# rasd3/TODA

Measured on AMD Instinct MI355X. Metric: LiDAR training samples/sec, higher is better.
Workload: dtype f32

## Files before the change

toda_amd/csrc/spconv.hip:

```cpp
#include <stdlib.h>

#include <type_traits>

#include <hip/hip_ext.h>

#include <mutex>
#include <vector>

#include "bn_fold.cuh"
#include "common.h"


namespace toda {

typedef float f32x4 __attribute__((ext_vector_type(4)));

constexpr int SC_BLOCK = 256;

static int tiles_pow2(int channels) {
    int t = (channels + 15) / 16, p = 1;
    while (p < t) p <<= 1;
    return p;
}

__global__ void __launch_bounds__(SC_BLOCK)
pack_weight_kernel(const float* __restrict__ w, int cout, int K, int cin, int transpose, int flip_k, int Q, int NT,
                   float* __restrict__ wp) {
    const long long e = (long long)blockIdx.x * SC_BLOCK + threadIdx.x;
    const long long total = (long long)K * Q * NT * 256;
    if (e >= total) return;
    const int j = (int)(e & 3);
    const int lane = (int)((e >> 2) & 63);
    long long t = e >> 8;
    const int n = (int)(t % NT);
    t /= NT;
    const int q = (int)(t % Q);
    const int k = (int)(t / Q);
    const int c = lane & 15, g = lane >> 4;
    const int gch = 16 * q + 4 * g + j;
    const int pch = NT * c + n;
    const int kk = flip_k ? K - 1 - k : k;
    float v = 0.0f;
    if (!transpose) {
        if (gch < cin && pch < cout) v = w[((size_t)pch * K + kk) * cin + gch];
    } else {
        if (gch < cout && pch < cin) v = w[((size_t)gch * K + kk) * cin + pch];
    }
    wp[e] = v;
}

constexpr int PACK_MAX_SEG = 48;
struct PackBatch {
    const float* w[PACK_MAX_SEG];
    float* wp[PACK_MAX_SEG];
    int cout[PACK_MAX_SEG], K[PACK_MAX_SEG], cin[PACK_MAX_SEG];
    unsigned char transpose[PACK_MAX_SEG], flip[PACK_MAX_SEG], Q[PACK_MAX_SEG], NT[PACK_MAX_SEG];
};

__global__ void __launch_bounds__(SC_BLOCK)
pack_weight_batch_kernel(const PackBatch b) {
    const int sg = blockIdx.y;
    const int K = b.K[sg], Q = b.Q[sg], NT = b.NT[sg], cin = b.cin[sg], cout = b.cout[sg];
    const long long e = (long long)blockIdx.x * SC_BLOCK + threadIdx.x;
// ... 951 lines not shown
    PackBatch b = {};
    toda::SplitPackBatch sb = {};
    int m = 0, sm = 0;
    long long most = 0, smost = 0;
    auto flush = [&]() -> int {
        if (m > 0) {
            hipLaunchKernelGGL(pack_weight_batch_kernel, dim3(cdiv(most, SC_BLOCK), m), dim3(SC_BLOCK), 0, (hipStream_t)stream, b);
            TODA_LAUNCH_CHECK();
        }
        m = 0, most = 0;
        return TODA_OK;
    };
    auto sflush = [&]() -> int {
        if (sm > 0) {
            hipLaunchKernelGGL(split_pack_batch_kernel, dim3(cdiv(smost, SC_BLOCK), sm), dim3(SC_BLOCK), 0, (hipStream_t)stream, sb);
            TODA_LAUNCH_CHECK();
        }
        sm = 0, smost = 0;
        return TODA_OK;
    };
    for (int s = 0; s < n; ++s) {
        TODA_CHECK_ARG(w[s] && wp[s] && cout[s] >= 1 && cin[s] >= 1 && k_vol[s] >= 1, "pack_weights: bad segment %d", s);
        const int cgather = transpose[s] ? cout[s] : cin[s], cprod = transpose[s] ? cin[s] : cout[s];
        TODA_CHECK_ARG(cgather <= 128 && cprod <= 128, "pack_weights: channels > 128 unsupported (segment %d)", s);
        if (use_split(cgather, cprod)) {
            split_pack_fill(sb, sm, w[s], cout[s], k_vol[s], cin[s], transpose[s], flip_k[s], wp[s]);
            const long long total = (long long)k_vol[s] * sb.KC[sm] * sb.NT[sm] * 192;
            if (total > smost) smost = total;
            if (++sm == toda::SPLIT_PACK_MAX_SEG) {
                const int rc = sflush();
                if (rc != TODA_OK) return rc;
            }
            continue;
        }
        const int i = m;
        b.w[i] = w[s], b.wp[i] = wp[s], b.cout[i] = cout[s], b.K[i] = k_vol[s], b.cin[i] = cin[s];
        b.transpose[i] = transpose[s] != 0, b.flip[i] = flip_k[s] != 0;
        b.Q[i] = (unsigned char)tiles_pow2(cgather), b.NT[i] = (unsigned char)tiles_pow2(cprod);
        const long long total = (long long)k_vol[s] * b.Q[i] * b.NT[i] * 256;
        if (total > most) most = total;
        if (++m == PACK_MAX_SEG) {
            const int rc = flush();
            if (rc != TODA_OK) return rc;
        }
    }
    {
        const int rc = flush();
        if (rc != TODA_OK) return rc;
    }
    return sflush();
}

namespace toda {
constexpr int CLS_ROWS = 8192, CLS_PER = CLS_ROWS / 256;
struct ClassGeom {
    int stride[3], pad[3];
};
__global__ void __launch_bounds__(256)
class_order_kernel(const int4* __restrict__ coords, int n, const ClassGeom gm, int32_t* __restrict__ order, unsigned char* __restrict__ cls_sorted) {
    __shared__ int cnt[8][256 + 1];
    const int base = blockIdx.x * CLS_ROWS, t = threadIdx.x;
    unsigned char c[CLS_PER];
    int mine[8] = {0, 0, 0, 0, 0, 0, 0, 0};
#pragma unroll
    for (int i = 0; i < CLS_PER; ++i) {
        const int r = base + t * CLS_PER + i;
        int cl = 0;
        if (r < n) {
            const int4 v = coords[r];
            cl = (((v.y + gm.pad[0]) % gm.stride[0]) * gm.stride[1] + (v.z + gm.pad[1]) % gm.stride[1]) * gm.stride[2] + (v.w + gm.pad[2]) % gm.stride[2];
            ++mine[cl & 7];
        }
        c[i] = (unsigned char)cl;
    }
#pragma unroll
    for (int k = 0; k < 8; ++k) cnt[k][t] = mine[k];
    __syncthreads();
    if (t < 8) {
        int run = 0;
        for (int j = 0; j < 256; ++j) {
            const int v = cnt[t][j];
            cnt[t][j] = run;
            run += v;
        }
        cnt[t][256] = run;
    }
    __syncthreads();
    int cls_base[8], run = 0;
#pragma unroll
    for (int k = 0; k < 8; ++k) {
        cls_base[k] = run + cnt[k][t];
        run += cnt[k][256];
    }
#pragma unroll
    for (int i = 0; i < CLS_PER; ++i) {
        const int r = base + t * CLS_PER + i;
        if (r >= n) break;
        const int k = c[i] & 7;
        int pos = 0;
#pragma unroll
        for (int q = 0; q < 8; ++q)
            if (q == k) pos = cls_base[q]++;
        order[base + pos] = r;
        cls_sorted[base + pos] = c[i];
    }
}

static int class_table(const int32_t* ksize, const int32_t* stride, const int32_t* pad, GatherClasses* out) {
    const int n_class = stride[0] * stride[1] * stride[2];
    if (n_class < 1 || n_class > 8 || ksize[0] * ksize[1] * ksize[2] > 27) return -1;
    *out = GatherClasses{};
    for (int rz = 0; rz < stride[0]; ++rz)
        for (int ry = 0; ry < stride[1]; ++ry)
            for (int rx = 0; rx < stride[2]; ++rx) {
                const int c = (rz * stride[1] + ry) * stride[2] + rx;
                int m = 0;
                for (int kz = 0; kz < ksize[0]; ++kz)
                    for (int ky = 0; ky < ksize[1]; ++ky)
                        for (int kx = 0; kx < ksize[2]; ++kx)
                            if (kz % stride[0] == rz && ky % stride[1] == ry && kx % stride[2] == rx)
                                out->k[c][m++] = (unsigned char)((kz * ksize[1] + ky) * ksize[2] + kx);
                out->count[c] = (unsigned char)m;
            }
    return 0;
}
}

extern "C" int toda_rulebook_class_order(const int32_t* in_coords, int n_in, const int32_t* stride, const int32_t* padding, int32_t* order,
                                         unsigned char* cls_sorted, void* stream) {
    TODA_CHECK_ARG(in_coords && stride && padding && order && cls_sorted && n_in >= 0, "rulebook_class_order: null argument");
    ClassGeom gm;
    for (int a = 0; a < 3; ++a) {
        TODA_CHECK_ARG(stride[a] >= 1 && stride[a] <= 2 && padding[a] >= 0, "rulebook_class_order: stride 1 or 2 per axis (got %d)", stride[a]);
        gm.stride[a] = stride[a], gm.pad[a] = padding[a];
    }
    if (n_in == 0) return TODA_OK;
    hipLaunchKernelGGL(class_order_kernel, dim3(cdiv(n_in, CLS_ROWS)), dim3(256), 0, (hipStream_t)stream, (const int4*)in_coords, n_in, gm, order,
                       cls_sorted);
    TODA_LAUNCH_CHECK();
    return TODA_OK;
}

namespace toda {
struct LaunchTimer {
    std::vector<hipEvent_t> ev;
    int used = 0;
    bool on = false;
};
static LaunchTimer g_timer;
static std::mutex g_timer_mu;
static inline void timer_next(hipEvent_t* start, hipEvent_t* stop) {
    *start = *stop = nullptr;
    if (!g_timer.on) return;
    std::lock_guard<std::mutex> lock(g_timer_mu);
    if (!g_timer.on || 2 * (g_timer.used + 1) > (int)g_timer.ev.size()) return;
    *start = g_timer.ev[2 * g_timer.used];
    *stop = g_timer.ev[2 * g_timer.used + 1];
    g_timer.used++;
}
}

#define GG_LAUNCH(kernel, grid, block, shmem, stream, ...)                                              \
    do {                                                                                               \
        hipEvent_t t0_, t1_;                                                                           \
        toda::timer_next(&t0_, &t1_);                                                                  \
        hipExtLaunchKernelGGL(kernel, grid, block, shmem, stream, t0_, t1_, 0, __VA_ARGS__);           \
    } while (0)

extern "C" int toda_timing_begin(int capacity) {
    TODA_CHECK_ARG(capacity > 0 && capacity <= (1 << 20), "timing_begin: capacity in (0, 2^20]");
    std::lock_guard<std::mutex> lock(toda::g_timer_mu);
    for (hipEvent_t e : g_timer.ev) (void)hipEventDestroy(e);
    g_timer.ev.assign((size_t)2 * capacity, nullptr);
    for (auto& e : g_timer.ev) TODA_HIP(hipEventCreate(&e));
    g_timer.used = 0;
    g_timer.on = true;
    return TODA_OK;
}

extern "C" int toda_timing_end(float* ms_out, int cap, int* n_out) {
    std::lock_guard<std::mutex> lock(toda::g_timer_mu);
    g_timer.on = false;
    const int n = g_timer.used < cap ? g_timer.used : cap;
    for (int i = 0; i < n; ++i) {
        TODA_HIP(hipEventSynchronize(g_timer.ev[2 * i + 1]));
        TODA_HIP(hipEventElapsedTime(&ms_out[i], g_timer.ev[2 * i], g_timer.ev[2 * i + 1]));
    }
    if (n_out) *n_out = g_timer.used;
    for (hipEvent_t e : g_timer.ev) (void)hipEventDestroy(e);
    g_timer.ev.clear();
// ... 28 lines not shown
    int rt, block, grid;
    bool vec;
};
}

static int gather_route(int c_gather, int c_produce, int n_out, bool stats, bool cls_sorted, GatherRoute* r) {
    const int Q = tiles_pow2(c_gather), NT = tiles_pow2(c_produce);
    const bool vec_ok = (c_gather & 3) == 0;
    const bool lds_faster = Q >= 2 && NT >= Q;
    r->rt = 2, r->block = SC_BLOCK, r->vec = vec_ok;
    if (use_split(c_gather, c_produce)) {
        TODA_CHECK_ARG(!(cls_sorted && stats), "gather_gemm (split path): no statistics on a class-sorted launch");
        r->family = GatherRoute::SPLIT;
    } else if (vec_ok && Q == 8 && NT == 8 && !cls_sorted) {
        r->family = GatherRoute::LDS_128, r->rt = 1, r->block = 512;
    } else if ((lds_faster || stats) && !cls_sorted && vec_ok && Q * NT <= 32) {
        r->family = GatherRoute::LDS, r->rt = NT < 8 ? 2 : 1;
    } else {
        TODA_CHECK_ARG(!stats, "gather_gemm: statistics requested on a launch shape without the fused epilogue");
        TODA_CHECK_ARG(vec_ok || Q == 1, "gather_gemm: gathered channel counts above 16 must be multiples of 4 (got %d)", c_gather);
        r->family = GatherRoute::REG;
        r->rt = NT < 8 ? 2 : (Q < 8 ? 1 : 2);
    }
    r->grid = cdiv(cdiv(n_out, 16 * r->rt), r->block / 64);
    return TODA_OK;
}

static int gather_gemm_impl(const float* in, int n_in, int c_gather, const float* wp, const int32_t* nbr, int n_out, int k_vol,
                            int c_produce, const float* bias, float* out, const int32_t* order, double* stats, int* blocks_out, void* stream,
                            const unsigned char* cls_sorted = nullptr, const toda::GatherClasses* cls_table = nullptr) {
    toda::GatherClasses classes = {};
    if (cls_sorted && cls_table) classes = *cls_table;
    else cls_sorted = nullptr;
    TODA_CHECK_ARG(c_gather >= 1 && c_gather <= 128 && c_produce >= 1 && c_produce <= 128,
                   "gather_gemm: channels must be in [1,128] (gather %d, produce %d)", c_gather, c_produce);
    TODA_CHECK_ARG(n_out >= 0 && n_in >= 0 && k_vol >= 1, "gather_gemm: bad sizes");
    TODA_CHECK_ARG((unsigned long long)n_in * c_gather * 4ull < 0xFFFFFFF0ull, "gather_gemm: gathered table must be < 4 GiB");
    if (n_out == 0) return TODA_OK;
    if (n_in == 0) {
        TODA_CHECK_ARG(bias == nullptr, "gather_gemm: empty input with bias is unsupported");
        TODA_HIP(hipMemsetAsync(out, 0, (size_t)n_out * c_produce * sizeof(float), (hipStream_t)stream));
        return TODA_OK;
    }
    GatherRoute r;
    const int rc = gather_route(c_gather, c_produce, n_out, stats != nullptr, cls_sorted != nullptr, &r);
    if (rc != TODA_OK) return rc;
    hipStream_t s = (hipStream_t)stream;
    const dim3 grid(r.grid), block(r.block);
    switch (r.family) {
        case GatherRoute::SPLIT:
            with_tiles(c_gather / 32, c_produce / 16, [&](auto kc, auto nt) {
                constexpr int KC = decltype(kc)::value, NT = decltype(nt)::value;
                if constexpr (KC <= 4 && NT >= 2)
                    GG_LAUNCH(HIP_KERNEL_NAME(gg_split_kernel<KC, NT, (NT == 8 ? 3 : 4), (NT == 2)>), grid, block, 0, s, in, n_in,
                              reinterpret_cast<const toda::u32x4*>(wp), nbr, n_out, k_vol, c_produce, bias, out, order, stats, cls_sorted, classes);
            });
            break;
        case GatherRoute::LDS_128:
            GG_LAUNCH(HIP_KERNEL_NAME(gather_gemm_lds_kernel<8, 8, 1, true, false, 512>), grid, block, 0, s, in, n_in, c_gather, wp, nbr, n_out,
                      k_vol, c_produce, bias, out, order, stats);
            break;
        case GatherRoute::LDS:
            with_tiles(tiles_pow2(c_gather), tiles_pow2(c_produce), [&](auto q, auto nt) {
                constexpr int Q = decltype(q)::value, NT = decltype(nt)::value, RT = NT < 8 ? 2 : 1;
                GG_LAUNCH(HIP_KERNEL_NAME(gather_gemm_lds_kernel<Q, NT, RT, true, true, SC_BLOCK, (Q <= 4 && NT <= 4 && RT == 2)>), grid, block, 0,
                          s, in, n_in, c_gather, wp, nbr, n_out, k_vol, c_produce, bias, out, order, stats);
            });
            break;
        case GatherRoute::REG: {
            auto reg = [&](auto q, auto nt, auto rt, auto vec) {
                constexpr int Q = decltype(q)::value, NT = decltype(nt)::value, RT = decltype(rt)::value;
                constexpr bool VEC = decltype(vec)::value;
                if (cls_sorted && VEC)
                    GG_LAUNCH(HIP_KERNEL_NAME(gather_gemm_kernel<Q, NT, RT, true, true>), grid, block, 0, s, in, n_in, c_gather, wp, nbr, n_out,
                              k_vol, c_produce, bias, out, order, cls_sorted, classes);
                else
                    GG_LAUNCH(HIP_KERNEL_NAME(gather_gemm_kernel<Q, NT, RT, VEC>), grid, block, 0, s, in, n_in, c_gather, wp, nbr, n_out, k_vol,
                              c_produce, bias, out, order, nullptr, classes);
            };
            if (!r.vec) {
                with_tiles(tiles_pow2(c_produce), [&](auto nt) {
                    reg(tile_c<1>{}, nt, tile_c<(decltype(nt)::value < 8 ? 2 : 1)>{}, std::false_type{});
                });
            } else {
                with_tiles(tiles_pow2(c_gather), tiles_pow2(c_produce), [&](auto q, auto nt) {
                    if constexpr (decltype(nt)::value < 8) reg(q, nt, tile_c<2>{}, std::true_type{});
                    else if (r.rt == 2) reg(q, nt, tile_c<2>{}, std::true_type{});
                    else reg(q, nt, tile_c<1>{}, std::true_type{});
                });
            }
            break;
        }
    }
    TODA_LAUNCH_CHECK();
    if (stats) {
        if (blocks_out) {
            *blocks_out = r.grid;
        } else {
            hipLaunchKernelGGL(toda::fold_partials_kernel, dim3(2 * c_produce), dim3(256), 0, s, stats, r.grid, 2 * c_produce);
            TODA_LAUNCH_CHECK();
        }
    }
    return TODA_OK;
}

extern "C" int toda_spconv_gather_gemm_ordered(const float* in, int n_in, int c_gather, const float* wp, const int32_t* nbr,
                                               int n_out, int k_vol, int c_produce, const float* bias, float* out,
// ... 176 lines not shown
```

toda_amd/csrc/spconv_split.cuh:

```cuda
#pragma once
#include "split_common.cuh"

namespace toda {

#ifndef WGS_ACCS
#define WGS_ACCS 2
#endif
#ifndef SP_STAMPS
#define SP_STAMPS 0
#endif
#if SP_STAMPS
#define SP_STAMP(i)                                                                               \
    do {                                                                                          \
        unsigned long long t_;                                                                    \
        __builtin_amdgcn_sched_barrier(0);                                                        \
        asm volatile("s_memtime %0\n\ts_waitcnt lgkmcnt(0)" : "=s"(t_)::"memory");                \
        __builtin_amdgcn_sched_barrier(0);                                                        \
        seg[i] += t_ - t_prev;                                                                    \
        t_prev = t_;                                                                              \
    } while (0)
#else
#define SP_STAMP(i)
#endif
#ifndef SP_ABLATE
// ... 28 lines not shown
    term(ah, bl);
    term(am, bm);
    term(am, bh);
    term(ah, bm);
    term(ah, bh);
}
__device__ __forceinline__ unsigned short sp_plane_of(float v, int plane) {
    const float h = sp_trunc(v), r = v - h, m = sp_trunc(r), l = r - m;
    const float pick = plane == 0 ? h : (plane == 1 ? m : l);
    return (unsigned short)(__builtin_bit_cast(unsigned, pick) >> 16);
}

constexpr int SPLIT_PACK_MAX_SEG = 48;
struct SplitPackBatch {
    const float* w[SPLIT_PACK_MAX_SEG];
    u32x4* wps[SPLIT_PACK_MAX_SEG];
    int cout[SPLIT_PACK_MAX_SEG], K[SPLIT_PACK_MAX_SEG], cin[SPLIT_PACK_MAX_SEG];
    unsigned char transpose[SPLIT_PACK_MAX_SEG], flip[SPLIT_PACK_MAX_SEG], KC[SPLIT_PACK_MAX_SEG], NT[SPLIT_PACK_MAX_SEG];
};
__global__ void __launch_bounds__(SC_BLOCK)
split_pack_batch_kernel(const SplitPackBatch b) {
    const int sg = blockIdx.y;
    const int K = b.K[sg], KC = b.KC[sg], NT = b.NT[sg], cin = b.cin[sg], cout = b.cout[sg];
    const long long e = (long long)blockIdx.x * SC_BLOCK + threadIdx.x;
    if (e >= (long long)K * KC * NT * 192) return;
    const int lane = (int)(e & 63);
    long long t = e >> 6;
    const int plane = (int)(t % 3);
    t /= 3;
    const int n = (int)(t % NT);
    t /= NT;
    const int kc = (int)(t % KC);
    const int k = (int)(t / KC);
    const int c = lane & 15, g = lane >> 4;
    const int pch = NT * c + n;
    const int kk = b.flip[sg] ? K - 1 - k : k;
    const float* __restrict__ w = b.w[sg];
    unsigned short v[8];
#pragma unroll
    for (int j = 0; j < 8; ++j) {
        const int gch = 32 * kc + 16 * (j >> 2) + 4 * g + (j & 3);
        float x = 0.0f;
        if (!b.transpose[sg]) {
            if (gch < cin && pch < cout) x = w[((size_t)pch * K + kk) * cin + gch];
        } else {
            if (gch < cout && pch < cin) x = w[((size_t)gch * K + kk) * cin + pch];
        }
        v[j] = sp_plane_of(x, plane);
    }
    b.wps[sg][e] = u32x4{(unsigned)v[0] | ((unsigned)v[1] << 16), (unsigned)v[2] | ((unsigned)v[3] << 16), (unsigned)v[4] | ((unsigned)v[5] << 16),
                         (unsigned)v[6] | ((unsigned)v[7] << 16)};
}

template <int KC, int NT, int WAVES, bool IL = false>
__global__ void __launch_bounds__(SC_BLOCK, WAVES)
gg_split_kernel(const float* __restrict__ in, int n_in, const u32x4* __restrict__ wps, const int* __restrict__ nbr, int n_out, int K, int cp,
                const float* __restrict__ bias, float* __restrict__ out, const int* __restrict__ order, double* __restrict__ stats,
                const unsigned char* __restrict__ cls_sorted, const GatherClasses classes) {
    constexpr int RT = 2;
    constexpr int CG = 32 * KC;
    constexpr int UNITS = NT * 3;
    constexpr int SLICE = UNITS * 64;
    static_assert(2 * SLICE * 16 >= (SC_BLOCK / 64) * 2 * 16 * NT * 4, "the statistics scratch aliases the weight buffers");
    __shared__ u32x4 wl[2 * SLICE];
    const int lane = threadIdx.x & 63, wv = threadIdx.x >> 6;
    const int blk = xcd_chunked_block(blockIdx.x, gridDim.x);
    const int wave = blk * (SC_BLOCK / 64) + wv;
    const int r = lane & 15, g = lane >> 4;
    const int row0 = wave * (16 * RT);

    f32x4 acc[RT][NT];
    int rows[RT];
    bool live[RT];
    gg_prologue<RT, NT>(bias, cp, row0, n_out, order, r, acc, rows, live);
    const __amdgpu_buffer_rsrc_t in_rsrc = table_rsrc(in, (unsigned)n_in * (unsigned)CG * 4u);
    int KE = K;
    bool listed = false;
    unsigned long long kpack = 0;
    if (cls_sorted) {
        const int p = row0 + (lane & (16 * RT - 1));
        const int c = cls_sorted[p < n_out ? p : n_out - 1], c0 = __builtin_amdgcn_readfirstlane(c);
        const bool same = __all(c == c0 || p >= n_out);
        int* cw = reinterpret_cast<int*>(wl);
        if (lane == 0) cw[wv] = same ? c0 : -1;
        __syncthreads();
        int cb = cw[0];
#pragma unroll
        for (int w = 1; w < SC_BLOCK / 64; ++w) cb = (cw[w] == cb) ? cb : -1;
        __syncthreads();
        if (cb >= 0 && classes.count[cb & 7] > 0 && classes.count[cb & 7] <= 8) {
            listed = true;
            KE = classes.count[cb & 7];
#pragma unroll
            for (int i = 0; i < 8; ++i) kpack |= (unsigned long long)classes.k[cb & 7][i] << (8 * i);
            kpack = ((unsigned long long)__builtin_amdgcn_readfirstlane((int)(kpack >> 32)) << 32) | (unsigned)__builtin_amdgcn_readfirstlane((int)kpack);
        }
    }
    auto kof = [&](int j) { return listed ? (int)((kpack >> (8 * j)) & 0xFF) : j; };
    auto load_ids = [&](int j, int (&dst)[RT]) {
        const int kk = kof(j < KE ? j : KE - 1);
#pragma unroll
        for (int rt = 0; rt < RT; ++rt) {
            dst[rt] = __builtin_nontemporal_load(nbr + (size_t)kk * n_out + rows[rt]);
        }
    };
    auto gather_rt = [&](const int (&src)[RT], int part, bool valid, f32x4 (&raw)[RT][2], int rt) {
        const bool ok = src[rt] >= 0 && valid;
        const unsigned base = (unsigned)src[rt] * (unsigned)(CG * 4) + (unsigned)(16 * g) + 128u * (unsigned)part;
#pragma unroll
        for (int i = 0; i < 2; ++i)
            raw[rt][i] = __builtin_bit_cast(f32x4, __builtin_amdgcn_raw_buffer_load_b128(in_rsrc, ok ? base + 64u * i : OOB, 0, 0));
    };
    auto gather = [&](const int (&src)[RT], int part, bool valid, f32x4 (&raw)[RT][2]) {
#pragma unroll
        for (int rt = 0; rt < RT; ++rt) gather_rt(src, part, valid, raw, rt);
    };
    auto stage = [&](int st, int buf) {
        const int sc = st < KE * KC ? st : KE * KC - 1;
        const int ss = kof(sc / KC) * KC + sc % KC;
#pragma unroll
        for (int t = 0; t < (UNITS + SC_BLOCK / 64 - 1) / (SC_BLOCK / 64); ++t) {
            const int u = t * (SC_BLOCK / 64) + wv;
            if (UNITS % (SC_BLOCK / 64) == 0 || u < UNITS)
                __builtin_amdgcn_global_load_lds(reinterpret_cast<const float*>(wps + (size_t)ss * SLICE + u * 64 + lane),
                                                 reinterpret_cast<float*>(&wl[buf * SLICE + u * 64]), 16, 0, 0);
        }
    };

    int idA[RT], idB[RT], idC[RT];
    f32x4 raw[RT][2];
    load_ids(0, idA);
    load_ids(1, idB);
    stage(0, 0);
    gather(idA, 0, true, raw);
    __syncthreads();

#if SP_STAMPS
    unsigned long long seg[6] = {0, 0, 0, 0, 0, 0}, t_prev;
    asm volatile("s_memtime %0\n\ts_waitcnt lgkmcnt(0)" : "=s"(t_prev)::"memory");
#endif
    auto body = [&](int k, const int (&ids_cur)[RT], const int (&ids_nxt)[RT], int (&ids_new)[RT]) {
        SP_STAMP(5);
        bool any = false;
#pragma unroll
        for (int rt = 0; rt < RT; ++rt) any = any || __any(ids_cur[rt] >= 0);
#pragma unroll
        for (int part = 0; part < KC; ++part) {
            const int cur = (k * KC + part) & 1;
            u32x4 ah[RT], am[RT], al[RT];
            f32x4 (&rw)[RT][2] = raw;
            if (any) {
#pragma unroll
                for (int rt = 0; rt < RT; ++rt) sp_split8(rw[rt][0], rw[rt][1], ah[rt], am[rt], al[rt]);
            }
            SP_STAMP(0);
            if constexpr (IL) {
                constexpr int PIECES = RT + 2;
                auto piece = [&](int p) {
                    if (p == 0) {
#if !(SP_ABLATE & 4)
                        stage(k * KC + part + 1, cur ^ 1);
#endif
                    } else if (p <= RT) {
                        if (part + 1 < KC) gather_rt(ids_cur, part + 1, true, raw, p - 1);
                        else gather_rt(ids_nxt, 0, k + 1 < KE, raw, p - 1);
                    } else if (part == KC - 1) load_ids(k + 2, ids_new);
                    asm volatile("" ::: "memory");
                };
                if (any) {
                    const u32x4* __restrict__ wb = wl + cur * SLICE + lane;
#pragma unroll
                    for (int n = 0; n < NT; ++n) {
                        const bf16x8 bh = __builtin_bit_cast(bf16x8, wb[(n * 3 + 0) * 64]), bm = __builtin_bit_cast(bf16x8, wb[(n * 3 + 1) * 64]),
                                     bl = __builtin_bit_cast(bf16x8, wb[(n * 3 + 2) * 64]);
#pragma unroll
                        for (int p = 0; p < PIECES; ++p)
                            if (p * NT / PIECES == n) piece(p);
                        sp_six_terms<false>(acc, n, ah, am, al, bh, bm, bl);
                    }
                } else {
#pragma unroll
                    for (int p = 0; p < PIECES; ++p) piece(p);
                }
            } else {
#if !(SP_ABLATE & 4)
            stage(k * KC + part + 1, cur ^ 1);
#endif
            asm volatile("" ::: "memory");
#if SP_ABLATE & 8
            if (k < 0)
#endif
            if (part + 1 < KC) gather(ids_cur, part + 1, true, raw);
            else gather(ids_nxt, 0, k + 1 < KE, raw);
            asm volatile("" ::: "memory");
#if !(SP_ABLATE & 16)
            if (part == KC - 1) load_ids(k + 2, ids_new);
#endif
            asm volatile("" ::: "memory");
            SP_STAMP(1);
            if (any) {
                const u32x4* __restrict__ wb = wl + cur * SLICE + lane;
#pragma unroll
                for (int n = 0; n < NT; ++n) {
                    const bf16x8 bh = __builtin_bit_cast(bf16x8, wb[(n * 3 + 0) * 64]), bm = __builtin_bit_cast(bf16x8, wb[(n * 3 + 1) * 64]),
                                 bl = __builtin_bit_cast(bf16x8, wb[(n * 3 + 2) * 64]);
                    sp_six_terms<(SP_ABLATE & 2) != 0>(acc, n, ah, am, al, bh, bm, bl);
                }
            }
            }
            SP_STAMP(2);
#if SP_ABLATE & (4 | 8 | 16)
            asm volatile("s_waitcnt vmcnt(0)" ::: "memory");
#else
            if (part == KC - 1) asm volatile("s_waitcnt vmcnt(%0)" ::"n"(RT * 2 + RT) : "memory");
            else asm volatile("s_waitcnt vmcnt(%0)" ::"n"(RT * 2) : "memory");
#endif
            SP_STAMP(3);
            __builtin_amdgcn_s_barrier();
            SP_STAMP(4);
        }
    };
    for (int k = 0;;) {
        body(k, idA, idB, idC);
        if (++k >= KE) break;
        body(k, idB, idC, idA);
        if (++k >= KE) break;
        body(k, idC, idA, idB);
        if (++k >= KE) break;
    }
    asm volatile("s_waitcnt vmcnt(0)" ::: "memory");
    if (row0 >= n_out && !stats) return;

#if SP_STAMPS
    if (stats) {
        if (lane == 0)
            for (int i = 0; i < 6; ++i) reinterpret_cast<unsigned long long*>(stats)[(size_t)wave * 6 + i] = seg[i];
        stats = nullptr;
    }
#endif
    if (stats) gg_moments<NT, RT, SC_BLOCK / 64>(reinterpret_cast<float (*)[2][16 * NT]>(wl), wv, blk, acc, row0, n_out, cp, stats, r, g);
    gg_store_rows<RT, NT>(acc, rows, row0, n_out, cp, out, r, g);
}

template <int MTB, int NTB, int QM = 1, int QN = 1>
__global__ void __launch_bounds__(SC_BLOCK, (MTB * NTB <= 4) ? 4 : ((MTB == 4 && NTB == 2) ? 3 : 2))
wgrad_split_kernel(const float* __restrict__ in, int n_in, const float* __restrict__ dout, const int* __restrict__ nbr, int n_out, int K,
                   int rows_per_chunk, float* __restrict__ slab) {
    static_assert((MTB == 2 || MTB == 4) && (NTB == 2 || NTB == 4), "32 or 64 channels a side");
    static_assert(QM * QN == 1 || (MTB == 4 && NTB == 4), "quarters are 64 x 64");
    static_assert(QM * QN == 1 || QM * QN == 2 || QM * QN == 4, "1, 2 or 4 quarters");
    constexpr int NQ = QM * QN, TEAMS = (SC_BLOCK / 64) / NQ;
    constexpr int MT = MTB * QM, NT = NTB * QN;
    constexpr int cin = 16 * MT, cout = 16 * NT;
    constexpr int QCAP = 64 + 32;
    __shared__ float red[TEAMS == 1 ? 1 : NQ * MTB * NTB * 4 * 64];
    __shared__ int q_in[SC_BLOCK / 64][QCAP], q_out[SC_BLOCK / 64][QCAP];
    const int lane = threadIdx.x & 63, wv = threadIdx.x >> 6;
    const int ii = lane & 15, g = lane >> 4;
    int chunk, k;
    wg_block(K, chunk, k);
    const int row_begin = chunk * rows_per_chunk;
    if (row_begin >= n_out) return;
    const int row_end = min(n_out, row_begin + rows_per_chunk);
    int* qi = q_in[wv];
    int* qo = q_out[wv];

    f32x4 acc[MTB][NTB];
#if WGS_ACCS >= 2
    f32x4 acc_s[MTB][NTB];
#endif
#if WGS_ACCS >= 3
    f32x4 acc_m[MTB][NTB];
#endif
#pragma unroll
    for (int m = 0; m < MTB; ++m)
#pragma unroll
        for (int n = 0; n < NTB; ++n) {
            acc[m][n] = f32x4{0.f, 0.f, 0.f, 0.f};
#if WGS_ACCS >= 2
            acc_s[m][n] = f32x4{0.f, 0.f, 0.f, 0.f};
#endif
// ... 77 lines not shown
            WS_TERM(acc_m, ah, bm);
            WS_TERM(acc, ah, bh);
#endif
#undef WS_TERM
        }
    };

    wg_pair_walk<32>(qi, qo, row_begin + team * 64, row_end, TEAMS * 64, nbr + (size_t)k * n_out, n_out, row_a, row_b, lane, std::true_type{}, round32);
#if WGS_ACCS >= 2
#pragma unroll
    for (int m = 0; m < MTB; ++m)
#pragma unroll
        for (int n = 0; n < NTB; ++n) {
#if WGS_ACCS >= 3
            acc[m][n] = (acc_s[m][n] + acc_m[m][n]) + acc[m][n];
#else
            acc[m][n] = acc_s[m][n] + acc[m][n];
#endif
        }
#endif

    for (int src = 1; src < TEAMS; ++src) {
        float* const rq = red + qd * (MTB * NTB * 4 * 64);
        if (team == src) {
#pragma unroll
            for (int m = 0; m < MTB; ++m)
#pragma unroll
                for (int n = 0; n < NTB; ++n)
#pragma unroll
                    for (int reg = 0; reg < 4; ++reg) rq[((m * NTB + n) * 4 + reg) * 64 + lane] = acc[m][n][reg];
        }
        __syncthreads();
        if (team == 0) {
#pragma unroll
            for (int m = 0; m < MTB; ++m)
#pragma unroll
                for (int n = 0; n < NTB; ++n)
#pragma unroll
                    for (int reg = 0; reg < 4; ++reg) acc[m][n][reg] += rq[((m * NTB + n) * 4 + reg) * 64 + lane];
        }
        __syncthreads();
    }
    if (team != 0) return;
    wg_store_slab<false>(acc, slab, chunk, k, K, MT, NT, m0, n0, cin, cout, ii, g);
}

static inline bool wgrad_split_shape_ok(int cin, int cout) {
    return ((cin == 32 || cin == 64) && (cout == 32 || cout == 64)) || ((cin == 64 || cin == 128) && (cout == 64 || cout == 128));
}

static inline bool split_shape_ok(int c_gather, int c_produce) {
    return (c_gather == 32 || c_gather == 64 || c_gather == 128) && (c_produce == 32 || c_produce == 64 || c_produce == 128);
}
static inline size_t split_packed_bytes(int k_vol, int c_gather, int c_produce) {
    return (size_t)k_vol * (c_gather / 32) * (c_produce / 16) * 3 * 1024;
}

}
```

toda_amd/csrc/rulebook.hip:

```cpp
#include "grid_index.cuh"
#include "scan.cuh"

namespace toda {

constexpr int RB_BLOCK = GI_TILE;

__global__ void __launch_bounds__(RB_BLOCK)
gi_mark_coords_kernel(const int4* __restrict__ idx, int n, const int32_t* __restrict__ n_dev, GridDims g,
                      uint2* __restrict__ cells) {
    n = eff_n(n, n_dev);
    const int i = blockIdx.x * RB_BLOCK + threadIdx.x;
    if (i >= n) return;
    const int4 c = idx[i];
    if (!in_grid(c, g)) return;
    gi_set_bit_first(cells, lin_index(c.x, c.y, c.z, c.w, g));
}

__global__ void __launch_bounds__(RB_BLOCK)
gi_rowof_kernel(const int4* __restrict__ idx, int n, const int32_t* __restrict__ n_dev, GridDims g,
                const uint2* __restrict__ cells, int* __restrict__ rowof) {
    n = eff_n(n, n_dev);
    const int i = blockIdx.x * RB_BLOCK + threadIdx.x;
    if (i >= n) return;
    const int4 c = idx[i];
// ... 440 lines not shown
static int conv_setup(const char* who, int batch, const int32_t* shape_in, const int32_t* ks, const int32_t* st, const int32_t* pd,
                      const int32_t* shape_out, const void* gi_out, GiView* out, ConvGeom* cg) {
    int rc = gi_view(who, gi_out, batch, shape_out, out);
    if (rc) return rc;
    for (int a = 0; a < 3; ++a) {
        TODA_CHECK_ARG(ks[a] >= 1 && st[a] >= 1 && pd[a] >= 0, "%s: bad kernel/stride/pad on axis %d", who, a);
        TODA_CHECK_ARG(shape_in[a] + 2 * pd[a] >= ks[a], "%s: axis %d of %d cells (+ 2 * %d) is shorter than the kernel's %d", who, a,
                       shape_in[a], pd[a], ks[a]);
        const int expect = (shape_in[a] + 2 * pd[a] - ks[a]) / st[a] + 1;
        TODA_CHECK_ARG(shape_out[a] == expect, "%s: shape_out[%d]=%d but (in+2p-k)/s+1=%d", who, a, shape_out[a], expect);
        cg->ks[a] = ks[a];
        cg->st[a] = st[a];
        cg->pd[a] = pd[a];
    }
    TODA_CHECK_ARG(ks[0] * ks[1] * ks[2] <= 64, "%s: kernel volume > 64 unsupported", who);
    cg->out = out->dims;
    return TODA_OK;
}

}

using namespace toda;

extern "C" size_t toda_gridindex_bytes(int batch, const int32_t* shape_host) {
    return gi_layout(batch, shape_host).bytes;
}

extern "C" int toda_gridindex_from_coords(const int32_t* idx, int n, const int32_t* n_dev, int batch,
                                          const int32_t* shape_host, void* gi, int32_t* rowof, void* stream) {
    hipStream_t s = (hipStream_t)stream;
    GiView v;
    int rc = gi_view("gridindex_from_coords", gi, batch, shape_host, &v);
    if (rc) return rc;
    TODA_CHECK_ARG(n >= 0, "gridindex_from_coords: n < 0");
    TODA_HIP(hipMemsetAsync(v.cells, 0, (size_t)v.n_cells * sizeof(uint2), s));
    const dim3 grid(cdiv(n, RB_BLOCK)), block(RB_BLOCK);
    if (n > 0) hipLaunchKernelGGL(gi_mark_coords_kernel, grid, block, 0, s, (const int4*)idx, n, n_dev, v.dims, v.cells);
    rc = exclusive_scan(CellAccess{v.cells}, v.n_cells, v.part, v.total, s);
    if (rc) return rc;
    if (n > 0 && rowof)
        hipLaunchKernelGGL(gi_rowof_kernel, grid, block, 0, s, (const int4*)idx, n, n_dev, v.dims, (const uint2*)v.cells, rowof);
    TODA_LAUNCH_CHECK();
    return TODA_OK;
}

extern "C" int toda_gridindex_from_coords_unordered(const int32_t* idx, int n, const int32_t* n_dev, int batch,
                                                    const int32_t* shape_host, void* gi, int32_t* rowof, int gi_clean,
                                                    void* stream) {
    hipStream_t s = (hipStream_t)stream;
    GiView v;
    int rc = gi_view("gridindex_from_coords_unordered", gi, batch, shape_host, &v);
    if (rc) return rc;
    TODA_CHECK_ARG(n >= 0 && rowof, "gridindex_from_coords_unordered: n < 0 or no rowof");
    if (!gi_clean) {
        TODA_HIP(hipMemsetAsync(v.cells, 0, (size_t)v.n_cells * sizeof(uint2), s));
        TODA_HIP(hipMemsetAsync(v.rowmask, 0, (size_t)v.n_rows, s));
    }
    if (n == 0) return TODA_OK;
    const dim3 grid(cdiv(n, RB_BLOCK)), block(RB_BLOCK);
    hipLaunchKernelGGL(gi_mark_first_kernel, grid, block, 0, s, (const int4*)idx, n, n_dev, v.dims, v.cells, v.rowmask, rowof, v.total);
    hipLaunchKernelGGL(gi_alloc_kernel, dim3(cdiv(n, GA_BLOCK)), dim3(GA_BLOCK), 0, s, (const int4*)idx, n, n_dev, v.dims, v.cells,
                       (const int*)rowof, v.total);
    hipLaunchKernelGGL(gi_rowof_kernel, grid, block, 0, s, (const int4*)idx, n, n_dev, v.dims, (const uint2*)v.cells, rowof);
    TODA_LAUNCH_CHECK();
    return TODA_OK;
}

extern "C" int toda_gridindex_clear(const int32_t* idx, int n, const int32_t* n_dev, int batch, const int32_t* shape_host,
                                    void* gi, void* stream) {
    GiView v;
    int rc = gi_view("gridindex_clear", gi, batch, shape_host, &v);
    if (rc) return rc;
    TODA_CHECK_ARG(n >= 0, "gridindex_clear: n < 0");
    if (n == 0) return TODA_OK;
    hipLaunchKernelGGL(gi_clear_kernel, dim3(cdiv(n, RB_BLOCK)), dim3(RB_BLOCK), 0, (hipStream_t)stream, (const int4*)idx, n, n_dev,
                       v.dims, v.cells, v.rowmask);
    TODA_LAUNCH_CHECK();
    return TODA_OK;
}

extern "C" int toda_gridindex_from_conv(const int32_t* idx_in, int n_in, const int32_t* n_in_dev, int batch,
                                        const int32_t* shape_in_host, const int32_t* ksize_host,
                                        const int32_t* stride_host, const int32_t* pad_host,
                                        const int32_t* shape_out_host, void* gi_out, int32_t* idx_out,
                                        int32_t* n_out_dev, int out_cap, void* stream) {
    hipStream_t s = (hipStream_t)stream;
    GiView v;
    ConvGeom cg;
    int rc = conv_setup("gridindex_from_conv", batch, shape_in_host, ksize_host, stride_host, pad_host, shape_out_host, gi_out, &v, &cg);
    if (rc) return rc;
    TODA_CHECK_ARG(n_in >= 0 && out_cap >= 0, "gridindex_from_conv: negative size");
    TODA_HIP(hipMemsetAsync(v.cells, 0, (size_t)v.n_cells * sizeof(uint2), s));
    if (n_in > 0)
        hipLaunchKernelGGL(gi_mark_conv_kernel, dim3(cdiv(n_in, RB_BLOCK)), dim3(RB_BLOCK), 0, s, (const int4*)idx_in,
                           n_in, n_in_dev, cg, v.cells);
    rc = exclusive_scan(CellAccess{v.cells}, v.n_cells, v.part, v.total, s);
    if (rc) return rc;
    hipLaunchKernelGGL(gi_decode_kernel, dim3(cdiv(v.n_cells, RB_BLOCK)), dim3(RB_BLOCK), 0, s, (const uint2*)v.cells, v.n_cells, v.dims,
                       (int4*)idx_out, out_cap, (const int32_t*)v.total, n_out_dev);
    TODA_LAUNCH_CHECK();
    return TODA_OK;
}

extern "C" int toda_gridindex_from_bitmap(const void* gi_in, int batch, const int32_t* shape_in_host,
                                          const int32_t* ksize_host, const int32_t* stride_host, const int32_t* pad_host,
                                          const int32_t* shape_out_host, void* gi_out, int32_t* idx_out, int32_t* n_out_dev,
                                          int out_cap, int in_rows_marked, void* stream) {
    hipStream_t s = (hipStream_t)stream;
    GiView in, out;
    ConvGeom cg;
// ... 73 lines not shown
```

Baseline: 149.1.

## Pack neighbor-id loads for two offsets into one load and skip empty gathers

The split gather-GEMM kernel now loads neighbor ids for two kernel offsets in a single per-lane load, using lane halves for each offset, and redistributes them with ds_bpermute. This halves the number of index vector-memory instructions, and the vmcnt wait counts are recomputed to match. For the KC=2/NT=2 shape it also skips issuing row gathers when no lane has a valid neighbor, and it raises occupancy for NT=2 to five waves per SIMD. The cost is extra LDS permute traffic with an lgkmcnt wait, a more intricate rotation of id buffers, and tighter register budgets.

```diff
diff --git a/toda_amd/csrc/spconv.hip b/toda_amd/csrc/spconv.hip
--- a/toda_amd/csrc/spconv.hip
+++ b/toda_amd/csrc/spconv.hip
@@ -1284,7 +1284,7 @@
             with_tiles(c_gather / 32, c_produce / 16, [&](auto kc, auto nt) {
                 constexpr int KC = decltype(kc)::value, NT = decltype(nt)::value;
                 if constexpr (KC <= 4 && NT >= 2)
-                    GG_LAUNCH(HIP_KERNEL_NAME(gg_split_kernel<KC, NT, (NT == 8 ? 3 : 4), (NT == 2)>), grid, block, 0, s, in, n_in,
+                    GG_LAUNCH(HIP_KERNEL_NAME(gg_split_kernel<KC, NT, (NT == 8 ? 3 : (NT == 2 ? 5 : 4)), (NT == 2), toda::split_vmem_mode(KC, NT)>), grid, block, 0, s, in, n_in,
                               reinterpret_cast<const toda::u32x4*>(wp), nbr, n_out, k_vol, c_produce, bias, out, order, stats, cls_sorted, classes);
             });
             break;
diff --git a/toda_amd/csrc/spconv_split.cuh b/toda_amd/csrc/spconv_split.cuh
--- a/toda_amd/csrc/spconv_split.cuh
+++ b/toda_amd/csrc/spconv_split.cuh
@@ -104,12 +104,17 @@
                          (unsigned)v[6] | ((unsigned)v[7] << 16)};
 }
 
-template <int KC, int NT, int WAVES, bool IL = false>
+constexpr int sp_vm_behind(int rt, bool packed, bool rows, bool ids) {
+    return (rows ? 2 * rt : 0) + (ids ? (packed ? 1 : rt) : 0);
+}
+template <int KC, int NT, int WAVES, bool IL = false, int VM = 0>
 __global__ void __launch_bounds__(SC_BLOCK, WAVES)
 gg_split_kernel(const float* __restrict__ in, int n_in, const u32x4* __restrict__ wps, const int* __restrict__ nbr, int n_out, int K, int cp,
                 const float* __restrict__ bias, float* __restrict__ out, const int* __restrict__ order, double* __restrict__ stats,
                 const unsigned char* __restrict__ cls_sorted, const GatherClasses classes) {
     constexpr int RT = 2;
+    constexpr bool PK = (VM & 1) != 0, SK = (VM & 2) != 0;
+    static_assert(!PK || RT == 2, "a packed id load is two offsets x two tiles x 16 rows");
     constexpr int CG = 32 * KC;
     constexpr int UNITS = NT * 3;
     constexpr int SLICE = UNITS * 64;
@@ -149,11 +154,39 @@
         }
     }
     auto kof = [&](int j) { return listed ? (int)((kpack >> (8 * j)) & 0xFF) : j; };
-    auto load_ids = [&](int j, int (&dst)[RT]) {
-        const int kk = kof(j < KE ? j : KE - 1);
-#pragma unroll
-        for (int rt = 0; rt < RT; ++rt) {
-            dst[rt] = __builtin_nontemporal_load(nbr + (size_t)kk * n_out + rows[rt]);
+    using IdSet = int[PK ? 1 : RT];
+    const int prow = rows[(lane >> 4) & (RT - 1)];
+    auto load_ids = [&](int j, IdSet& dst) {
+        if constexpr (PK) {
+            const int k0 = kof(j < KE ? j : KE - 1), k1 = kof(j + 1 < KE ? j + 1 : KE - 1);
+            dst[0] = __builtin_nontemporal_load(nbr + (size_t)((lane & 32) ? k1 : k0) * n_out + prow);
+        } else {
+            const int kk = kof(j < KE ? j : KE - 1);
+#pragma unroll
+            for (int rt = 0; rt < RT; ++rt) dst[rt] = __builtin_nontemporal_load(nbr + (size_t)kk * n_out + rows[rt]);
+        }
+    };
+    auto ids_any = [&](const IdSet& s, auto half_tag) {
+        if constexpr (PK) {
+            const unsigned long long b = __ballot(s[0] >= 0);
+            return (unsigned)(decltype(half_tag)::value ? b >> 32 : b) != 0u;
+        } else {
+            bool any = false;
+#pragma unroll
+            for (int rt = 0; rt < RT; ++rt) any = any || __any(s[rt] >= 0);
+            return any;
+        }
+    };
+    auto ids_get = [&](const IdSet& s, auto half_tag, int (&dst)[RT]) {
+        if constexpr (PK) {
+            constexpr int H = decltype(half_tag)::value;
+            const int lane4 = 4 * r, packed = s[0];
+            asm volatile("ds_bpermute_b32 %0, %2, %3 offset:%4\n\tds_bpermute_b32 %1, %2, %3 offset:%5\n\ts_waitcnt lgkmcnt(0)"
+                         : "=&v"(dst[0]), "=&v"(dst[1])
+                         : "v"(lane4), "v"(packed), "n"(128 * H), "n"(128 * H + 64));
+        } else {
+#pragma unroll
+            for (int rt = 0; rt < RT; ++rt) dst[rt] = s[rt];
         }
     };
     auto gather_rt = [&](const int (&src)[RT], int part, bool valid, f32x4 (&raw)[RT][2], int rt) {
@@ -179,23 +212,33 @@
         }
     };
 
-    int idA[RT], idB[RT], idC[RT];
+    constexpr std::integral_constant<int, 0> LOWER{};
+    constexpr std::integral_constant<int, 1> UPPER{};
+    IdSet idA, idB, idC;
+    int idc[RT];
+    bool have;
     f32x4 raw[RT][2];
     load_ids(0, idA);
-    load_ids(1, idB);
+    if constexpr (!PK) load_ids(1, idB);
     stage(0, 0);
-    gather(idA, 0, true, raw);
+    have = ids_any(idA, LOWER);
+    ids_get(idA, LOWER, idc);
+    if (!SK || have) gather(idc, 0, true, raw);
     __syncthreads();
 
 #if SP_STAMPS
     unsigned long long seg[6] = {0, 0, 0, 0, 0, 0}, t_prev;
     asm volatile("s_memtime %0\n\ts_waitcnt lgkmcnt(0)" : "=s"(t_prev)::"memory");
 #endif
-    auto body = [&](int k, const int (&ids_cur)[RT], const int (&ids_nxt)[RT], int (&ids_new)[RT]) {
+    auto wait_slice = [&](bool rows_req, auto ids_tag) {
+        constexpr bool IDS = decltype(ids_tag)::value;
+        if (rows_req) asm volatile("s_waitcnt vmcnt(%0)" ::"n"(sp_vm_behind(RT, PK, true, IDS)) : "memory");
+        else asm volatile("s_waitcnt vmcnt(%0)" ::"n"(sp_vm_behind(RT, PK, false, IDS)) : "memory");
+    };
+    auto body = [&](int k, const IdSet& nxt, auto half, IdSet& fresh, auto load_tag) {
+        constexpr bool LOAD = decltype(load_tag)::value;
         SP_STAMP(5);
-        bool any = false;
-#pragma unroll
-        for (int rt = 0; rt < RT; ++rt) any = any || __any(ids_cur[rt] >= 0);
+        const bool any = have;
 #pragma unroll
         for (int part = 0; part < KC; ++part) {
             const int cur = (k * KC + part) & 1;
@@ -206,17 +249,28 @@
                 for (int rt = 0; rt < RT; ++rt) sp_split8(rw[rt][0], rw[rt][1], ah[rt], am[rt], al[rt]);
             }
             SP_STAMP(0);
+            const bool last = part == KC - 1;
+            bool want = any;
+            auto next_rows = [&]() {
+                if (!last) return;
+                want = k + 1 < KE && ids_any(nxt, half);
+                if (!SK || want) ids_get(nxt, half, idc);
+            };
+            auto request_rt = [&](int rt) {
+                if (SK && !want) return;
+                gather_rt(idc, last ? 0 : part + 1, SK || !last || k + 1 < KE, raw, rt);
+            };
             if constexpr (IL) {
                 constexpr int PIECES = RT + 2;
                 auto piece = [&](int p) {
                     if (p == 0) {
+                        next_rows();
 #if !(SP_ABLATE & 4)
                         stage(k * KC + part + 1, cur ^ 1);
 #endif
                     } else if (p <= RT) {
-                        if (part + 1 < KC) gather_rt(ids_cur, part + 1, true, raw, p - 1);
-                        else gather_rt(ids_nxt, 0, k + 1 < KE, raw, p - 1);
-                    } else if (part == KC - 1) load_ids(k + 2, ids_new);
+                        request_rt(p - 1);
+                    } else if (last && LOAD) load_ids(k + 2, fresh);
                     asm volatile("" ::: "memory");
                 };
                 if (any) {
@@ -235,6 +289,7 @@
                     for (int p = 0; p < PIECES; ++p) piece(p);
                 }
             } else {
+            next_rows();
 #if !(SP_ABLATE & 4)
             stage(k * KC + part + 1, cur ^ 1);
 #endif
@@ -242,11 +297,13 @@
 #if SP_ABLATE & 8
             if (k < 0)
 #endif
-            if (part + 1 < KC) gather(ids_cur, part + 1, true, raw);
-            else gather(ids_nxt, 0, k + 1 < KE, raw);
+            {
+#pragma unroll
+                for (int rt = 0; rt < RT; ++rt) request_rt(rt);
+            }
             asm volatile("" ::: "memory");
 #if !(SP_ABLATE & 16)
-            if (part == KC - 1) load_ids(k + 2, ids_new);
+            if (last && LOAD) load_ids(k + 2, fresh);
 #endif
             asm volatile("" ::: "memory");
             SP_STAMP(1);
@@ -264,21 +321,35 @@
 #if SP_ABLATE & (4 | 8 | 16)
             asm volatile("s_waitcnt vmcnt(0)" ::: "memory");
 #else
-            if (part == KC - 1) asm volatile("s_waitcnt vmcnt(%0)" ::"n"(RT * 2 + RT) : "memory");
-            else asm volatile("s_waitcnt vmcnt(%0)" ::"n"(RT * 2) : "memory");
+            if (last && LOAD) wait_slice(!SK || want, std::true_type{});
+            else wait_slice(!SK || want, std::false_type{});
 #endif
             SP_STAMP(3);
             __builtin_amdgcn_s_barrier();
             SP_STAMP(4);
-        }
-    };
+            if (last) have = want;
+        }
+    };
+    constexpr std::true_type LOADS{};
+    constexpr std::false_type RESTS{};
     for (int k = 0;;) {
-        body(k, idA, idB, idC);
-        if (++k >= KE) break;
-        body(k, idB, idC, idA);
-        if (++k >= KE) break;
-        body(k, idC, idA, idB);
-        if (++k >= KE) break;
+        if constexpr (PK) {
+            body(k, idA, UPPER, idB, LOADS);
+            if (++k >= KE) break;
+            body(k, idB, LOWER, idA, RESTS);
+            if (++k >= KE) break;
+            body(k, idB, UPPER, idA, LOADS);
+            if (++k >= KE) break;
+            body(k, idA, LOWER, idB, RESTS);
+            if (++k >= KE) break;
+        } else {
+            body(k, idB, LOWER, idC, LOADS);
+            if (++k >= KE) break;
+            body(k, idC, LOWER, idA, LOADS);
+            if (++k >= KE) break;
+            body(k, idA, LOWER, idB, LOADS);
+            if (++k >= KE) break;
+        }
     }
     asm volatile("s_waitcnt vmcnt(0)" ::: "memory");
     if (row0 >= n_out && !stats) return;
@@ -462,6 +533,13 @@
 static inline bool split_shape_ok(int c_gather, int c_produce) {
     return (c_gather == 32 || c_gather == 64 || c_gather == 128) && (c_produce == 32 || c_produce == 64 || c_produce == 128);
 }
+#ifndef SP_VM_FORCE
+#define SP_VM_FORCE -1
+#endif
+constexpr int split_vmem_mode(int kc, int nt) {
+    if (SP_VM_FORCE >= 0) return SP_VM_FORCE;
+    return (kc == 2 && nt == 2) ? 3 : 1;
+}
 static inline size_t split_packed_bytes(int k_vol, int c_gather, int c_produce) {
     return (size_t)k_vol * (c_gather / 32) * (c_produce / 16) * 3 * 1024;
 }
```

Result: no change. 149.0 (-0.1%).

## Rewrite class-order sort with wave ballots and block scan; merge grid-index memsets

Applied to the files above, without the earlier changes.

The class-order kernel now runs with 1024 threads and coalesced strided loads. It ranks each row within its wave using ballots and popcount, and computes per-(class, chunk) offsets with a block-wide exclusive scan instead of a serial 8-thread scan over 256 entries. Separately, the two memsets that clear the grid-index cells and rowmask are merged into one. The merged memset assumes rowmask sits contiguously after cells, and any padding between them is also zeroed.

```diff
diff --git a/toda_amd/csrc/rulebook.hip b/toda_amd/csrc/rulebook.hip
--- a/toda_amd/csrc/rulebook.hip
+++ b/toda_amd/csrc/rulebook.hip
@@ -516,10 +516,7 @@
     int rc = gi_view("gridindex_from_coords_unordered", gi, batch, shape_host, &v);
     if (rc) return rc;
     TODA_CHECK_ARG(n >= 0 && rowof, "gridindex_from_coords_unordered: n < 0 or no rowof");
-    if (!gi_clean) {
-        TODA_HIP(hipMemsetAsync(v.cells, 0, (size_t)v.n_cells * sizeof(uint2), s));
-        TODA_HIP(hipMemsetAsync(v.rowmask, 0, (size_t)v.n_rows, s));
-    }
+    if (!gi_clean) TODA_HIP(hipMemsetAsync(v.cells, 0, (size_t)((char*)(v.rowmask + v.n_rows) - (char*)v.cells), s));
     if (n == 0) return TODA_OK;
     const dim3 grid(cdiv(n, RB_BLOCK)), block(RB_BLOCK);
     hipLaunchKernelGGL(gi_mark_first_kernel, grid, block, 0, s, (const int4*)idx, n, n_dev, v.dims, v.cells, v.rowmask, rowof, v.total);
diff --git a/toda_amd/csrc/spconv.hip b/toda_amd/csrc/spconv.hip
--- a/toda_amd/csrc/spconv.hip
+++ b/toda_amd/csrc/spconv.hip
@@ -9,6 +9,7 @@
 
 #include "bn_fold.cuh"
 #include "common.h"
+#include "scan.cuh"
 
 
 namespace toda {
@@ -1066,57 +1067,51 @@
 }
 
 namespace toda {
-constexpr int CLS_ROWS = 8192, CLS_PER = CLS_ROWS / 256;
+constexpr int CLS_ROWS = 8192, CLS_BLOCK = 1024, CLS_PER = CLS_ROWS / CLS_BLOCK, CLS_CHUNKS = CLS_ROWS / 64;
+static_assert(8 * CLS_CHUNKS == CLS_BLOCK, "one (class, chunk) count per thread");
 struct ClassGeom {
     int stride[3], pad[3];
 };
-__global__ void __launch_bounds__(256)
+__device__ __forceinline__ unsigned long long class_lanes(int k, unsigned long long valid, unsigned long long b0, unsigned long long b1,
+                                                          unsigned long long b2) {
+    return valid & ((k & 1) ? b0 : ~b0) & ((k & 2) ? b1 : ~b1) & ((k & 4) ? b2 : ~b2);
+}
+__global__ void __launch_bounds__(CLS_BLOCK)
 class_order_kernel(const int4* __restrict__ coords, int n, const ClassGeom gm, int32_t* __restrict__ order, unsigned char* __restrict__ cls_sorted) {
-    __shared__ int cnt[8][256 + 1];
-    const int base = blockIdx.x * CLS_ROWS, t = threadIdx.x;
+    __shared__ int first[8 * CLS_CHUNKS];
+    const int base = blockIdx.x * CLS_ROWS, t = threadIdx.x, lane = t & 63, wave = t >> 6;
+    const unsigned long long below = (1ull << lane) - 1ull;
+    int4 v[CLS_PER];
+#pragma unroll
+    for (int i = 0; i < CLS_PER; ++i) {
+        const int r = base + i * CLS_BLOCK + t;
+        v[i] = r < n ? coords[r] : make_int4(0, 0, 0, 0);
+    }
     unsigned char c[CLS_PER];
-    int mine[8] = {0, 0, 0, 0, 0, 0, 0, 0};
+    int rank[CLS_PER];
 #pragma unroll
     for (int i = 0; i < CLS_PER; ++i) {
-        const int r = base + t * CLS_PER + i;
-        int cl = 0;
+        const bool live = base + i * CLS_BLOCK + t < n;
+        const int cl = (((v[i].y + gm.pad[0]) % gm.stride[0]) * gm.stride[1] + (v[i].z + gm.pad[1]) % gm.stride[1]) * gm.stride[2] +
+                       (v[i].w + gm.pad[2]) % gm.stride[2];
+        c[i] = (unsigned char)cl;
+        const unsigned long long valid = __ballot(live), b0 = __ballot(cl & 1), b1 = __ballot(cl & 2), b2 = __ballot(cl & 4);
+        rank[i] = __popcll(class_lanes(cl & 7, valid, b0, b1, b2) & below);
+        if (lane < 8) first[lane * CLS_CHUNKS + i * (CLS_BLOCK / 64) + wave] = __popcll(class_lanes(lane, valid, b0, b1, b2));
+    }
+    __syncthreads();
+    int total;
+    const int at = block_exclusive_scan<CLS_BLOCK>(first[t], &total);
+    first[t] = at;
+    __syncthreads();
+#pragma unroll
+    for (int i = 0; i < CLS_PER; ++i) {
+        const int r = base + i * CLS_BLOCK + t;
         if (r < n) {
-            const int4 v = coords[r];
-            cl = (((v.y + gm.pad[0]) % gm.stride[0]) * gm.stride[1] + (v.z + gm.pad[1]) % gm.stride[1]) * gm.stride[2] + (v.w + gm.pad[2]) % gm.stride[2];
-            ++mine[cl & 7];
-        }
-        c[i] = (unsigned char)cl;
-    }
-#pragma unroll
-    for (int k = 0; k < 8; ++k) cnt[k][t] = mine[k];
-    __syncthreads();
-    if (t < 8) {
-        int run = 0;
-        for (int j = 0; j < 256; ++j) {
-            const int v = cnt[t][j];
-            cnt[t][j] = run;
-            run += v;
-        }
-        cnt[t][256] = run;
-    }
-    __syncthreads();
-    int cls_base[8], run = 0;
-#pragma unroll
-    for (int k = 0; k < 8; ++k) {
-        cls_base[k] = run + cnt[k][t];
-        run += cnt[k][256];
-    }
-#pragma unroll
-    for (int i = 0; i < CLS_PER; ++i) {
-        const int r = base + t * CLS_PER + i;
-        if (r >= n) break;
-        const int k = c[i] & 7;
-        int pos = 0;
-#pragma unroll
-        for (int q = 0; q < 8; ++q)
-            if (q == k) pos = cls_base[q]++;
-        order[base + pos] = r;
-        cls_sorted[base + pos] = c[i];
+            const int pos = base + first[(c[i] & 7) * CLS_CHUNKS + i * (CLS_BLOCK / 64) + wave] + rank[i];
+            order[pos] = r;
+            cls_sorted[pos] = c[i];
+        }
     }
 }
 
@@ -1149,7 +1144,7 @@
         gm.stride[a] = stride[a], gm.pad[a] = padding[a];
     }
     if (n_in == 0) return TODA_OK;
-    hipLaunchKernelGGL(class_order_kernel, dim3(cdiv(n_in, CLS_ROWS)), dim3(256), 0, (hipStream_t)stream, (const int4*)in_coords, n_in, gm, order,
+    hipLaunchKernelGGL(class_order_kernel, dim3(cdiv(n_in, CLS_ROWS)), dim3(CLS_BLOCK), 0, (hipStream_t)stream, (const int4*)in_coords, n_in, gm, order,
                        cls_sorted);
     TODA_LAUNCH_CHECK();
     return TODA_OK;
```

Measured after the change: 149.9 before, 150.0 after, median of 2. About the same (+0.1%).
